# simonsysu/tfs

Measured on AMD Instinct MI355X. Metric: GiB/s CRC32 verify, device-resident 64 KiB files; 1/2/4/8 MI355X, higher is better.
Workload: dtype u8

## Files before the change

### tfs_amd/csrc/replicate_plan.h

```cpp
#pragma once
#include <algorithm>
#include <cstdint>
#include <vector>

#include "../../include/tfs_replicate.h"
#include "crc_math.h"

namespace tfscrc {

constexpr uint32_t kRepHead = 56;
constexpr uint32_t kRepOverhead = TFS_RAW_FRAME_OVERHEAD;
constexpr uint32_t kRepInfo = 36;
constexpr uint32_t kRepFlag = 0x4e534654u;
constexpr uint32_t kRepSeg = 16u << 10;
constexpr uint32_t kRepNoRec = 0xffffffffu;
constexpr int32_t kRepParameterError = -1016, kRepSizeError = -8034, kRepSizeInvalid = -16002;

struct RepUnit {
  uint64_t soff;
  uint64_t doff;
  uint32_t hlen;
  uint32_t hk;
  uint32_t plen;
  uint32_t rec;
  uint32_t frame;
  uint32_t mfh;
  uint32_t mfp;
  uint32_t mr;
};
static_assert(sizeof(RepUnit) == 48, "replicate unit layout");

struct RepFrame {
  uint64_t doff;
  uint64_t pid;
  uint32_t seed;
  uint32_t length;
  uint32_t offset;
  uint32_t flag;
  uint32_t block_id;
  uint32_t type_ver;
  uint32_t u0, nu;
};
static_assert(sizeof(RepFrame) == 48, "replicate frame layout");

struct RepRec {
  uint64_t file_id;
  int32_t offset, size;
};

struct RepPlan {
  int32_t total = 0, frame_len = 0;
  uint32_t nframes = 0;
  std::vector<RepUnit> units;
  std::vector<uint32_t> frame_first;
  std::vector<RepRec> recs;
  std::vector<uint32_t> index;
  std::vector<int32_t> early;
};

inline uint32_t rep_frame_count(int64_t total, int64_t frame_len) {
  if (total < 0 || frame_len <= 0) return 0u;
  return uint32_t(std::max<int64_t>(1, (total + frame_len - 1) / frame_len));
}

inline uint32_t rep_pow(uint64_t d) {
  struct Pow {
    uint32_t t[4][256];
    Pow() {
      for (int j = 0; j < 4; ++j) {
        t[j][0] = 1u << 31;
        const uint32_t step = shift_bytes_pow(1u << 31, uint64_t(1) << (8 * j));
        for (int v = 1; v < 256; ++v) t[j][v] = multmodp(t[j][v - 1], step);
      }
    }
  };
  static const Pow pw;
  uint32_t p = pw.t[0][d & 255u];
  for (int j = 1; j < 4; ++j)
    if ((d >> (8 * j)) & 255u) p = multmodp(p, pw.t[j][(d >> (8 * j)) & 255u]);
  return d >> 32 ? multmodp(p, shift_bytes_pow(1u << 31, d >> 32 << 32)) : p;
}

struct RepPowWalk {
  uint64_t d = 0;
  uint32_t m = 0;
  bool valid = false;
  uint32_t at(uint64_t nd) {
    struct Seg {
      uint32_t t[4][256];
      Seg() { make_shift_table(t, kRepSeg); }
    };
    static const Seg sg;
    if (valid && nd == d + kRepSeg)
      m = sg.t[0][m & 255u] ^ sg.t[1][(m >> 8) & 255u] ^ sg.t[2][(m >> 16) & 255u] ^ sg.t[3][m >> 24];
    else
      m = rep_pow(nd);
    d = nd, valid = true;
    return m;
  }
};

inline uint32_t rep_crc_bytes(uint32_t c, const uint8_t* p, uint32_t len) {
  for (uint32_t i = 0; i < len; ++i) {
    c ^= p[i];
    for (int k = 0; k < 8; ++k) c = (c & 1u) ? (c >> 1) ^ kPoly : (c >> 1);
  }
  return c;
}

inline void rep_le32(uint8_t* p, uint32_t v) {
  p[0] = uint8_t(v), p[1] = uint8_t(v >> 8), p[2] = uint8_t(v >> 16), p[3] = uint8_t(v >> 24);
}

inline void rep_info_bytes(uint32_t block_id, uint32_t offset, uint32_t length, uint8_t h[32]) {
  std::fill(h, h + 32, uint8_t(0));
  rep_le32(h, block_id);
  rep_le32(h + 12, offset);
  rep_le32(h + 16, length);
}

inline uint32_t rep_frame_seed(uint32_t block_id, uint32_t offset, uint32_t length, uint32_t flag) {
  uint8_t h[32], f[4];
  rep_info_bytes(block_id, offset, length, h);
  rep_le32(f, flag);
  return shift_bytes_pow(rep_crc_bytes(kRepFlag, h, 32), uint64_t(length) + 4u) ^ rep_crc_bytes(0u, f, 4);
}

inline int rep_cfg_status(const tfs_replicate_cfg& c) {
  if (c.total < 0 || c.frame_len <= 0 || c.frame_len % 1024 != 0) return kRepSizeInvalid;
  if (c.frame_stride != 0 && uint64_t(c.frame_stride) < uint64_t(c.frame_len) + kRepOverhead) return kRepParameterError;
  if (c.new_block != TFS_RAW_NORMAL_DATA && c.new_block != TFS_RAW_PARITY_DATA) return kRepParameterError;
  if (c.reserved != 0) return kRepParameterError;
  return 0;
}

inline uint64_t rep_stride(const tfs_replicate_cfg& c) {
  return c.frame_stride ? uint64_t(c.frame_stride) : uint64_t(c.frame_len) + kRepOverhead;
}

inline int make_replicate_plan(const tfs_replicate_cfg& c, const tfs_raw_meta* metas, uint32_t n, RepPlan* p) {
  *p = RepPlan();
  if (const int rc = rep_cfg_status(c)) return rc;
  if (n && !metas) return kRepParameterError;
  const int64_t total = c.total, fl = c.frame_len;
  p->total = c.total, p->frame_len = c.frame_len;
  p->nframes = rep_frame_count(total, fl);
  int64_t last_end = 0;
  for (uint32_t i = 0; i < n; ++i) {
    const tfs_raw_meta& m = metas[i];
    if (m.offset < 0 || int64_t(m.offset) + int64_t(m.size) > total) {
      p->early.push_back(kRepParameterError);
      continue;
    }
    if (m.size <= int32_t(kRepInfo)) {
      p->early.push_back(kRepSizeError);
      continue;
    }
    if (int64_t(m.offset) < last_end) return kRepParameterError;
    last_end = int64_t(m.offset) + int64_t(m.size);
    p->early.push_back(0);
    p->recs.push_back(RepRec{m.file_id, m.offset, m.size});
    p->index.push_back(i);
  }
  auto piece_end = [&](int64_t pos, int64_t end) {
    const int64_t fend = std::min<int64_t>((pos / fl + 1) * fl, total);
    int64_t e = std::min(end, fend);
    if (e - pos > int64_t(kRepSeg)) e = (pos / int64_t(kRepSeg) + 1) * int64_t(kRepSeg);
    return e;
  };
  auto push = [&](int64_t pos, uint32_t hlen, uint32_t hk, uint32_t plen, uint32_t rec, int64_t rec_end) {
    const int64_t fend = std::min<int64_t>((pos / fl + 1) * fl, total);
    const int64_t uend = pos + hlen + plen;
    RepUnit u{};
    u.soff = uint64_t(pos);
    u.hlen = hlen, u.hk = hk, u.plen = plen, u.rec = rec;
    u.frame = uint32_t(pos / fl);
    u.mfh = hlen ? rep_pow(uint64_t(fend - (pos + hlen)) + 4u) : 0u;
    u.mfp = uint32_t(fend - uend) + 4u;
    u.mr = rec == kRepNoRec ? 0u : uint32_t(rec_end - uend);
    p->units.push_back(u);
  };
  auto gap = [&](int64_t pos, int64_t end) {
    while (pos < end) {
      const int64_t e = piece_end(pos, end);
      push(pos, 0u, 0u, uint32_t(e - pos), kRepNoRec, 0);
      pos = e;
    }
  };
  int64_t pos = 0;
  for (uint32_t r = 0; r < uint32_t(p->recs.size()); ++r) {
    const int64_t off = p->recs[r].offset, info_end = off + kRepInfo, end = off + p->recs[r].size;
    gap(pos, off);
    pos = off;
    while (pos < end) {
      const int64_t fend = std::min<int64_t>((pos / fl + 1) * fl, total);
      uint32_t hlen = 0, hk = 0, plen = 0;
      const int64_t start = pos;
      if (pos < info_end) {
        hk = uint32_t(pos - off);
        hlen = uint32_t(std::min(info_end, fend) - pos);
        pos += hlen;
      }
      if (pos >= info_end && pos < fend) {
        plen = uint32_t(piece_end(pos, end) - pos);
        pos += plen;
      }
      push(start, hlen, hk, plen, r, end);
    }
  }
  gap(pos, total);
  RepPowWalk fw, rw;
  for (size_t k = p->units.size(); k-- > 0;) {
    RepUnit& u = p->units[k];
    u.mfp = fw.at(u.mfp);
    if (u.rec != kRepNoRec) u.mr = rw.at(u.mr);
  }
  p->frame_first.assign(size_t(p->nframes) + 1, uint32_t(p->units.size()));
  for (uint32_t k = uint32_t(p->units.size()); k-- > 0;) p->frame_first[p->units[k].frame] = k;
  for (uint32_t f = p->nframes; f-- > 0;)
    p->frame_first[f] = std::min(p->frame_first[f], p->frame_first[f + 1]);
  return 0;
}

inline bool rep_call_ok(const RepPlan& p, int64_t next, bool done, int64_t offset, int64_t len) {
  if (offset != next || len < 0) return false;
  if (p.total == 0) return !done && offset == 0 && len == 0;
  if (len == 0 || offset + len > p.total) return false;
  return offset % p.frame_len == 0 && (len % p.frame_len == 0 || offset + len == p.total);
}

inline uint32_t rep_call_frames(const RepPlan& p, int64_t len) {
  return uint32_t(std::max<int64_t>(1, (len + p.frame_len - 1) / p.frame_len));
}
inline uint64_t rep_call_need(const RepPlan& p, int64_t len, uint64_t stride) {
  const uint32_t nf = rep_call_frames(p, len);
  const uint64_t last = uint64_t(len) - uint64_t(nf - 1) * uint64_t(p.frame_len);
  return uint64_t(nf - 1) * stride + kRepOverhead + last;
}

inline uint32_t rep_slice_units(const RepPlan& p, uint32_t f0, uint32_t nf) {
  return p.frame_first[f0 + nf] - p.frame_first[f0];
}

inline void rep_make_slice(const RepPlan& p, const tfs_replicate_cfg& c, uint64_t stride, uint32_t f0, uint32_t nf,
                           RepFrame* frames, RepUnit* units) {
  const uint32_t ub = p.frame_first[f0];
  const uint64_t base = uint64_t(f0) * uint64_t(p.frame_len);
  for (uint32_t j = 0; j < nf; ++j) {
    const uint32_t f = f0 + j;
    const uint64_t off = uint64_t(f) * uint64_t(p.frame_len);
    RepFrame& fr = frames[j];
    fr.doff = uint64_t(j) * stride;
    fr.pid = c.packet_id + f;
    fr.length = uint32_t(std::min<uint64_t>(uint64_t(p.frame_len), uint64_t(p.total) - off));
    fr.offset = uint32_t(off);
    fr.flag = f == 0 ? uint32_t(int32_t(c.new_block)) : 0u;
    fr.block_id = c.block_id;
    fr.type_ver = uint32_t(TFS_WRITE_RAW_DATA_MESSAGE) | uint32_t(uint16_t(c.version)) << 16;
    fr.seed = rep_frame_seed(c.block_id, fr.offset, fr.length, fr.flag);
    fr.u0 = p.frame_first[f] - ub;
    fr.nu = p.frame_first[f + 1] - p.frame_first[f];
  }
  const uint32_t nu = rep_slice_units(p, f0, nf);
  for (uint32_t k = 0; k < nu; ++k) {
    RepUnit u = p.units[ub + k];
    const uint64_t pos = u.soff;
    const uint32_t j = u.frame - f0;
    u.soff = pos - base;
    u.doff = uint64_t(j) * stride + kRepHead + (pos - uint64_t(u.frame) * uint64_t(p.frame_len));
    u.frame = j;
    units[k] = u;
  }
}

}
```

### tfs_amd/csrc/tfs_crc_abi.cpp

```cpp
#include <emmintrin.h>
#include <hip/hip_runtime.h>

#include <algorithm>
#include <atomic>
#include <chrono>
#include <condition_variable>
#include <cstdarg>
#include <cstdio>
#include <cstdlib>
#include <cstring>
#include <map>
#include <memory>
#include <mutex>
#include <shared_mutex>
#include <string>
#include <vector>

#include "../../include/tfs_crc.h"
#include "../../include/tfs_crc_testing.h"
#include "../../include/tfs_read.h"
#include "../../include/tfs_replicate.h"
#include "../../include/tfs_write.h"
#include "crc_math.h"
#include "pin_registry.h"
// ... 204 lines not shown
  DevBuf d_src, d_dst, d_aux;
  PinBuf h_aux, h_status, h_stage;
  std::vector<uint32_t> live_idx;
  tfs_block_job* job = nullptr;
  std::vector<tfs_block_job*> gjobs;
  std::vector<uint32_t> gstart;
  std::vector<CompactJob> gjob_list;
  bool busy = false;
  void release() {
    d_src.release(); d_dst.release(); d_aux.release();
    h_aux.release(); h_status.release(); h_stage.release();
    if (done) (void)hipEventDestroy(done);
    if (stream) (void)hipStreamDestroy(stream);
    done = nullptr;
    stream = nullptr;
  }
};
struct ReadPlanSlot {
  PinBuf h;
  DevBuf d;
  hipEvent_t done = nullptr;
  void release() {
    if (done) {
      (void)hipEventSynchronize(done);
      (void)hipEventDestroy(done);
    }
    done = nullptr;
    h.release();
    d.release();
  }
};
constexpr uint32_t kReadPlanRing = 4;
struct RepRes {
  DevBuf d_cap, d_racc, d_fcrc, d_recs, d_res;
  PinBuf h_res, h_recs;
  ReadPlanSlot slots[4];
  hipEvent_t ready = nullptr;
  uint32_t slot_next = 0;
  void release() {
    for (auto& sl : slots) sl.release();
    d_cap.release(); d_racc.release(); d_fcrc.release(); d_recs.release(); d_res.release();
    h_res.release(); h_recs.release();
    if (ready) (void)hipEventDestroy(ready);
    ready = nullptr;
  }
};
constexpr size_t kRepPool = 8;
constexpr uint64_t kReadPiece = 32ull << 20;
constexpr int kCompactSlots = 8;
constexpr uint32_t kSchedSlots = 256;
constexpr uint32_t kForeignSlots = 64;
constexpr uint32_t kOwnedSlots = kSchedSlots - kForeignSlots;
constexpr int kVariantDmaCompact = 8;
#ifdef TFS_CRC_MEASURE
constexpr int kVariantStagedWide = 52;
constexpr int kVariantWideCtxStream = 53;
#else
constexpr int kVariantStagedWide = -1;
constexpr int kVariantWideCtxStream = -1;
#endif
constexpr int64_t kResRecentNs = 50'000'000;
constexpr uint64_t kZeroCopySpan = 8ull << 20;
constexpr uint32_t kZeroCopyOutFiles = 65536;

}

struct tfs_crc_ctx {
  int device = -1;
  uint64_t id = 0;
  hipStream_t stream = nullptr;
  hipStream_t lat_stream = nullptr;
  int lat_prio = 0;
  Tables* d_tables = nullptr;
  std::mutex mu;
// ... 2171 lines not shown
    HIP_TRY(ctx, hipMemcpyAsync(ctx->read_h_res.p, d_res, size_t(m) * sizeof(tfs_read_result), hipMemcpyDeviceToHost,
                                ctx->stream));
    HIP_TRY(ctx, hipStreamSynchronize(ctx->stream));
    const tfs_read_result* hr = static_cast<const tfs_read_result*>(ctx->read_h_res.p);
    for (uint32_t k = 0; k < m; ++k) {
      results[i0 + k] = hr[k];
      bad += hr[k].status != TFS_SUCCESS ? 1u : 0u;
      if (!out_zc && hr[k].frame_len)
        memcpy(o8 + jobs[i0 + k].frame_offset, static_cast<const uint8_t*>(ctx->read_h_out.p) + opos[k], hr[k].frame_len);
    }
    i0 = i1;
  }
  if (n_bad) *n_bad += bad;
  return bad ? TFS_EXIT_CHECK_CRC_ERROR : TFS_SUCCESS;
}

int tfs_read_set_piece(tfs_crc_ctx* ctx, uint64_t bytes) {
  if (!ctx) return TFS_EXIT_PARAMETER_ERROR;
  ctx->read_piece.store(bytes ? bytes : kReadPiece, std::memory_order_relaxed);
  return TFS_SUCCESS;
}


struct tfs_replicate {
  tfs_crc_ctx* ctx = nullptr;
  tfs_replicate_cfg cfg{};
  RepPlan plan;
  uint32_t n = 0;
  hipStream_t stream = nullptr;
  bool stream_set = false;
  int64_t next = 0;
  bool done = false;
  bool waited = false;
  std::unique_ptr<RepRes> r;
};

extern "C++" {
namespace {

int rep_call_checks(tfs_replicate* s, const void* src, int offset, int len, const void* out, uint64_t out_cap) {
  if (!s) return TFS_EXIT_PARAMETER_ERROR;
  if (!rep_call_ok(s->plan, s->next, s->done, offset, len))
    return set_err(s->ctx, TFS_EXIT_PARAMETER_ERROR, "replicate: call [%d, +%d) is not the next one (covered %lld of %d)",
                   offset, len, (long long)s->next, s->plan.total);
  if ((len > 0 && !src) || !out) return TFS_EXIT_DATA_INVALID;
  if (out_cap < rep_call_need(s->plan, len, rep_stride(s->cfg)))
    return set_err(s->ctx, TFS_EXIT_PARAMETER_ERROR, "replicate: out_cap does not hold the call's frames");
  return TFS_SUCCESS;
}

int rep_enqueue(tfs_replicate* s, hipStream_t st, const uint8_t* d_src, uint32_t f0, uint32_t nf, uint64_t src_len,
                uint8_t* d_out, uint64_t stride) {
  tfs_crc_ctx* ctx = s->ctx;
  RepRes& r = *s->r;
  ReadPlanSlot& rp = r.slots[r.slot_next++ % 4u];
  if (!s->waited) {
    if (st != ctx->stream) HIP_TRY(ctx, hipStreamWaitEvent(st, r.ready, 0));
    s->waited = true;
  }
  if (rp.done) HIP_TRY(ctx, hipEventSynchronize(rp.done));
  const uint32_t nu = rep_slice_units(s->plan, f0, nf);
  const size_t fbytes = size_t(nf) * sizeof(RepFrame), ubytes = size_t(nu) * sizeof(RepUnit);
  HIP_TRY(ctx, rp.h.reserve(fbytes + ubytes));
  HIP_TRY(ctx, rp.d.reserve(fbytes + ubytes + size_t(nu) * 8u));
  RepFrame* hf = static_cast<RepFrame*>(rp.h.p);
  RepUnit* hu = reinterpret_cast<RepUnit*>(static_cast<uint8_t*>(rp.h.p) + fbytes);
  rep_make_slice(s->plan, s->cfg, stride, f0, nf, hf, hu);
  uint8_t* d8 = static_cast<uint8_t*>(rp.d.p);
  const uint8_t* plan8 = static_cast<const uint8_t*>(rp.h.dev);
  if (!plan8) {
    HIP_TRY(ctx, hipMemcpyAsync(rp.d.p, rp.h.p, fbytes + ubytes, hipMemcpyHostToDevice, st));
    plan8 = d8;
  }
  SCHED_LAUNCH(ctx, st, "replicate",
               launch_replicate(d_src, src_len, reinterpret_cast<const RepUnit*>(plan8 + fbytes), nu,
                                reinterpret_cast<const RepFrame*>(plan8), nf, d_out, ctx->d_tables,
                                reinterpret_cast<uint32_t*>(d8 + fbytes + ubytes), static_cast<uint8_t*>(r.d_cap.p),
                                static_cast<uint32_t*>(r.d_racc.p), static_cast<uint32_t*>(r.d_fcrc.p) + f0, sched,
                                st, throughput_cap(ctx)));
  if (!rp.done) HIP_TRY(ctx, hipEventCreateWithFlags(&rp.done, hipEventDisableTiming));
  HIP_TRY(ctx, hipEventRecord(rp.done, st));
  return TFS_SUCCESS;
}

void rep_release(tfs_replicate* s) {
  if (!s->r) return;
  std::lock_guard<std::mutex> g(s->ctx->rep_mu);
  if (s->ctx->rep_pool.size() < kRepPool) s->ctx->rep_pool.push_back(std::move(s->r));
  else s->r->release();
  s->r.reset();
}

}
}

uint32_t tfs_replicate_frame_count(const tfs_replicate_cfg* cfg) {
  return cfg ? rep_frame_count(cfg->total, cfg->frame_len) : 0u;
}

int tfs_replicate_begin(tfs_crc_ctx* ctx, const tfs_replicate_cfg* cfg, const tfs_raw_meta* metas, uint32_t n,
                        tfs_replicate** out) {
  if (!ctx || !cfg || !out) return TFS_EXIT_PARAMETER_ERROR;
  *out = nullptr;
  std::unique_ptr<tfs_replicate> s(new tfs_replicate());
  if (const int rc = make_replicate_plan(*cfg, metas, n, &s->plan))
    return set_err(ctx, rc, "replicate begin: the configuration or the metas are refused (%d)", rc);
  s->ctx = ctx;
  s->cfg = *cfg;
  s->n = n;
  const size_t na = s->plan.recs.size();
  HIP_TRY(ctx, hipSetDevice(ctx->device));
  {
    std::lock_guard<std::mutex> g(ctx->rep_mu);
    if (!ctx->rep_pool.empty()) {
      s->r = std::move(ctx->rep_pool.back());
      ctx->rep_pool.pop_back();
    }
  }
  if (!s->r) s->r.reset(new RepRes());
  int rc = TFS_SUCCESS;
  auto setup = [&]() -> int {
    RepRes& r = *s->r;
    HIP_TRY(ctx, r.d_fcrc.reserve(size_t(s->plan.nframes) * 4u));
    HIP_TRY(ctx, r.h_res.reserve(na * 8u + size_t(s->plan.nframes) * 4u));
    if (!r.ready) HIP_TRY(ctx, hipEventCreateWithFlags(&r.ready, hipEventDisableTiming));
    if (na) {
      HIP_TRY(ctx, r.d_cap.reserve(na * kFileInfoSize));
      HIP_TRY(ctx, r.d_racc.reserve(na * 4u));
      HIP_TRY(ctx, r.d_recs.reserve(na * sizeof(RepRec)));
      HIP_TRY(ctx, r.h_recs.reserve(na * sizeof(RepRec)));
      HIP_TRY(ctx, r.d_res.reserve(na * 8u));
      memcpy(r.h_recs.p, s->plan.recs.data(), na * sizeof(RepRec));
    }
    std::lock_guard<std::mutex> g(ctx->mu);
    if (na) {
      HIP_TRY(ctx, hipMemsetAsync(r.d_racc.p, 0, na * 4u, ctx->stream));
      HIP_TRY(ctx, hipMemcpyAsync(r.d_recs.p, r.h_recs.p, na * sizeof(RepRec), hipMemcpyHostToDevice, ctx->stream));
    }
    HIP_TRY(ctx, hipEventRecord(r.ready, ctx->stream));
    return TFS_SUCCESS;
  };
  rc = setup();
  if (rc != TFS_SUCCESS) {
    rep_release(s.get());
    return rc;
  }
  *out = s.release();
  return TFS_SUCCESS;
}

int tfs_replicate_frames_device(tfs_replicate* s, const void* d_src, int offset, int len, void* d_out,
                                uint64_t out_cap, void* stream) {
  if (const int rc = rep_call_checks(s, d_src, offset, len, d_out, out_cap)) return rc;
  tfs_crc_ctx* ctx = s->ctx;
  hipStream_t st = stream ? static_cast<hipStream_t>(stream) : ctx->stream;
  if (st == hipStreamPerThread)
    return set_err(ctx, TFS_EXIT_PARAMETER_ERROR, "hipStreamPerThread is not accepted; pass NULL or a stream of your own");
  if (s->stream_set && st != s->stream)
    return set_err(ctx, TFS_EXIT_PARAMETER_ERROR, "replicate: one stream per session");
  HIP_TRY(ctx, hipSetDevice(ctx->device));
  const uint32_t f0 = uint32_t(offset / s->plan.frame_len), nf = rep_call_frames(s->plan, len);
  if (const int rc = rep_enqueue(s, st, static_cast<const uint8_t*>(d_src), f0, nf, uint64_t(len),
                                 static_cast<uint8_t*>(d_out), rep_stride(s->cfg)))
    return rc;
  s->stream = st, s->stream_set = true;
  s->next += len;
  s->done = true;
  return TFS_SUCCESS;
}

int tfs_replicate_frames(tfs_replicate* s, const void* src, int offset, int len, void* out, uint64_t out_cap) {
  if (const int rc = rep_call_checks(s, src, offset, len, out, out_cap)) return rc;
  tfs_crc_ctx* ctx = s->ctx;
  if (s->stream_set && s->stream != ctx->stream)
    return set_err(ctx, TFS_EXIT_PARAMETER_ERROR, "replicate: one stream per session");
  const uint32_t f0 = uint32_t(offset / s->plan.frame_len), nf = rep_call_frames(s->plan, len);
  {
    const Desc d0{0u, uint32_t(len), 0u};
    count_host_call(ctx, &d0, nf);
  }
  std::lock_guard<std::mutex> g(ctx->mu);
  if (const int f = injected_fault(ctx)) return f;
  HIP_TRY(ctx, hipSetDevice(ctx->device));
  void *zsrc = nullptr, *zout = nullptr;
  const bool src_zc = len == 0 || (is_pinned_host(src) && host_dev_ptr(src, &zsrc));
  const bool out_zc = is_pinned_host(out) && host_dev_ptr(out, &zout);
  (void)hipGetLastError();
  const uint64_t fl = uint64_t(s->plan.frame_len), ustride = rep_stride(s->cfg), sstride = fl + 64u;
  const uint8_t* s8 = static_cast<const uint8_t*>(src);
  uint8_t* o8 = static_cast<uint8_t*>(out);
  uint32_t per = nf;
  if (!src_zc || !out_zc) {
    const uint64_t piece = std::max<uint64_t>(ctx->read_piece.load(std::memory_order_relaxed), 1u);
    per = uint32_t(std::min<uint64_t>(nf, std::max<uint64_t>(piece / sstride, 1u)));
  }
  for (uint32_t j0 = 0; j0 < nf; j0 += per) {
    const uint32_t m = std::min(per, nf - j0);
    const uint64_t poff = uint64_t(j0) * fl;
    const uint64_t plen = std::min<uint64_t>(uint64_t(m) * fl, uint64_t(len) - poff);
    const uint8_t* d_src = static_cast<const uint8_t*>(zsrc) + poff;
// ... 5 lines not shown
      stride = sstride;
    }
    if (!src_zc) {
      HIP_TRY(ctx, ctx->read_h_src.reserve(plen + 16u));
      HIP_TRY(ctx, ctx->read_d_src.reserve(plen + 16u));
      const uintptr_t want = out_zc ? reinterpret_cast<uintptr_t>(d_out) + kRepHead : 0u;
      const uint64_t sa = (want - reinterpret_cast<uintptr_t>(ctx->read_d_src.p)) & 15u;
      memcpy(static_cast<uint8_t*>(ctx->read_h_src.p) + sa, s8 + poff, plen);
      if (plen)
        HIP_TRY(ctx, hipMemcpyAsync(static_cast<uint8_t*>(ctx->read_d_src.p) + sa,
                                    static_cast<uint8_t*>(ctx->read_h_src.p) + sa, plen, hipMemcpyHostToDevice,
                                    ctx->stream));
      d_src = static_cast<const uint8_t*>(ctx->read_d_src.p) + sa;
    }
    uint64_t oa = 0;
    if (!out_zc) {
      oa = (reinterpret_cast<uintptr_t>(d_src) - kRepHead - reinterpret_cast<uintptr_t>(ctx->read_d_out.p)) & 15u;
      d_out = static_cast<uint8_t*>(ctx->read_d_out.p) + oa;
    }
    if (const int rc = rep_enqueue(s, ctx->stream, d_src, f0 + j0, m, plen, d_out, stride)) return rc;
    const uint64_t last = plen - uint64_t(m - 1) * fl;
    if (!out_zc)
      HIP_TRY(ctx, hipMemcpyAsync(static_cast<uint8_t*>(ctx->read_h_out.p) + oa, d_out,
                                  uint64_t(m - 1) * sstride + kRepOverhead + last, hipMemcpyDeviceToHost, ctx->stream));
    HIP_TRY(ctx, hipStreamSynchronize(ctx->stream));
    if (!out_zc)
      for (uint32_t j = 0; j < m; ++j)
        memcpy(o8 + uint64_t(j0 + j) * ustride, static_cast<const uint8_t*>(ctx->read_h_out.p) + oa + uint64_t(j) * sstride,
               kRepOverhead + (j + 1 < m ? fl : last));
  }
  s->stream = ctx->stream, s->stream_set = true;
  s->next += len;
  s->done = true;
  return TFS_SUCCESS;
}

int tfs_replicate_finish(tfs_replicate* s, uint32_t* out_crc, int32_t* out_status, uint32_t* n_bad,
                         uint32_t* out_frame_crc) {
  if (!s) return TFS_EXIT_PARAMETER_ERROR;
  tfs_crc_ctx* ctx = s->ctx;
  if (!(s->plan.total == 0 ? s->done : s->next == s->plan.total))
    return set_err(ctx, TFS_EXIT_PARAMETER_ERROR, "replicate finish: %lld of %d bytes covered", (long long)s->next,
                   s->plan.total);
  HIP_TRY(ctx, hipSetDevice(ctx->device));
  hipStream_t st = s->stream_set ? s->stream : ctx->stream;
  const uint32_t na = uint32_t(s->plan.recs.size()), nfr = s->plan.nframes;
  RepRes& r = *s->r;
  if (!s->waited && st != ctx->stream) HIP_TRY(ctx, hipStreamWaitEvent(st, r.ready, 0));
  uint32_t* hr = static_cast<uint32_t*>(r.h_res.p);
  if (na) {
    uint32_t* d_crc = static_cast<uint32_t*>(r.d_res.p);
    HIP_TRY(ctx, launch_replicate_finish(static_cast<const RepRec*>(r.d_recs.p), na,
                                         static_cast<const uint8_t*>(r.d_cap.p),
                                         static_cast<const uint32_t*>(r.d_racc.p), d_crc,
                                         reinterpret_cast<int32_t*>(d_crc + na), st));
    HIP_TRY(ctx, hipMemcpyAsync(hr, d_crc, size_t(na) * 8u, hipMemcpyDeviceToHost, st));
  }
  HIP_TRY(ctx, hipMemcpyAsync(hr + 2u * size_t(na), r.d_fcrc.p, size_t(nfr) * 4u, hipMemcpyDeviceToHost, st));
  HIP_TRY(ctx, hipStreamSynchronize(st));
  uint32_t bad = 0;
  for (uint32_t i = 0; i < s->n; ++i) {
    if (out_crc) out_crc[i] = 0u;
    if (out_status) out_status[i] = s->plan.early[i];
    bad += s->plan.early[i] != 0 ? 1u : 0u;
  }
  for (uint32_t r = 0; r < na; ++r) {
    const int32_t status = int32_t(hr[na + r]);
    if (out_crc) out_crc[s->plan.index[r]] = hr[r];
    if (out_status) out_status[s->plan.index[r]] = status;
    bad += status != TFS_SUCCESS ? 1u : 0u;
  }
  if (out_frame_crc) memcpy(out_frame_crc, hr + 2u * size_t(na), size_t(nfr) * 4u);
  if (n_bad) *n_bad += bad;
  return TFS_SUCCESS;
}

int tfs_replicate_free(tfs_replicate* s) {
  if (!s) return TFS_EXIT_PARAMETER_ERROR;
  (void)hipSetDevice(s->ctx->device);
  if (s->stream_set) (void)hipStreamSynchronize(s->stream);
  if (!s->waited && s->r && s->r->ready) (void)hipEventSynchronize(s->r->ready);
  rep_release(s);
  delete s;
  return TFS_SUCCESS;
}


int tfs_crc32_shift_device(tfs_crc_ctx* ctx, const uint32_t* d_crc, const uint32_t* d_nbytes, uint32_t n,
                           uint32_t* d_out, void* stream) {
  if (!ctx || (n && (!d_crc || !d_nbytes || !d_out))) return TFS_EXIT_PARAMETER_ERROR;
  if (n == 0) return TFS_SUCCESS;
  HIP_TRY(ctx, hipSetDevice(ctx->device));
  hipStream_t st = stream ? static_cast<hipStream_t>(stream) : ctx->stream;
  HIP_TRY(ctx, launch_crc_shift(ctx->d_tables, d_crc, d_nbytes, n, d_out, st));
  return TFS_SUCCESS;
}

int tfs_crc32_synth_fill_device(tfs_crc_ctx* ctx, void* d_dst, uint64_t nbytes, uint64_t seed, uint64_t first_word,
                                void* stream) {
  if (!ctx || !d_dst || (nbytes & 7)) return TFS_EXIT_PARAMETER_ERROR;
  HIP_TRY(ctx, hipSetDevice(ctx->device));
  hipStream_t st = stream ? static_cast<hipStream_t>(stream) : ctx->stream;
  HIP_TRY(ctx, launch_synth_fill(static_cast<uint64_t*>(d_dst), nbytes / 8, seed, first_word, st));
  return TFS_SUCCESS;
}

int tfs_crc32_write_headers_device(tfs_crc_ctx* ctx, void* d_image, const uint64_t* d_rec_off, const uint32_t* d_len,
                                   const uint32_t* d_crc, uint64_t first_id, uint32_t n, void* stream) {
  if (!ctx || !d_image) return TFS_EXIT_PARAMETER_ERROR;
  HIP_TRY(ctx, hipSetDevice(ctx->device));
  hipStream_t st = stream ? static_cast<hipStream_t>(stream) : ctx->stream;
  HIP_TRY(ctx, launch_write_headers(static_cast<uint8_t*>(d_image), d_rec_off, d_len, d_crc, first_id, n, st));
  return TFS_SUCCESS;
// ... 382 lines not shown
```

### tfs_amd/csrc/tfs_crc_kernels.hip

```cpp
#include <hip/hip_runtime.h>
#include <stdint.h>

#include <type_traits>

#include "read_reply_plan.h"
#include "replicate_plan.h"
#include "tfs_crc_device.h"

namespace tfscrc {

typedef const __attribute__((address_space(1))) uint32_t* gu32p;
typedef unsigned int u32x4 __attribute__((ext_vector_type(4)));
typedef const __attribute__((address_space(1))) u32x4* gu128p;
typedef const __attribute__((address_space(1))) uint8_t* gu8p;
__device__ __forceinline__ uint32_t ld32(uintptr_t a) { return *reinterpret_cast<gu32p>(a); }
__device__ __forceinline__ uint4 ld128(uintptr_t a) {
  const u32x4 v = *reinterpret_cast<gu128p>(a);
  return make_uint4(v.x, v.y, v.z, v.w);
}
template <bool NT>
__device__ __forceinline__ uint4 ld128s(uintptr_t a) {
  if (NT) {
    const u32x4 v = __builtin_nontemporal_load(reinterpret_cast<gu128p>(a));
    return make_uint4(v.x, v.y, v.z, v.w);
  }
  return ld128(a);
}
__device__ __forceinline__ uint32_t ld8(uintptr_t a) { return *reinterpret_cast<gu8p>(a); }

__device__ __forceinline__ uint32_t xor3(uint32_t a, uint32_t b, uint32_t c) {
  return __builtin_amdgcn_bitop3_b32(a, b, c, 0x96);
}

__device__ __forceinline__ uint32_t lds_ld(const uint32_t* T, uint32_t byte_addr) {
  return *reinterpret_cast<const uint32_t*>(reinterpret_cast<const char*>(T) + byte_addr);
// ... 1920 lines not shown
      }
      if (uint32_t(lane) < cur.hlen) {
        out[cur.doff + uint32_t(lane)] = uint8_t(st.hb);
        cap[uint64_t(cur.rec) * kFileInfoSize + cur.hk + uint32_t(lane)] = uint8_t(st.hb);
      }
      if (st.g.nstripes) {
        if (lane == 0) {
          const uint32_t ntw = uint32_t((st.g.end & ~uintptr_t(3)) - st.g.B16) / 4u;
          for (uint32_t i = 0; i < 3u; ++i)
            if (i < ntw) st32u(st.g.B16 + 4u * i + st.delta, st.h.tw[i]);
          const uintptr_t B = st.g.end & ~uintptr_t(3);
          for (uint32_t i = 0; i < 3u; ++i)
            if (B + i < st.g.end) *reinterpret_cast<uint8_t*>(B + i + st.delta) = uint8_t(st.h.tb[i]);
        }
      } else {
        copy_unaligned(src + cur.soff + cur.hlen, out + cur.doff + cur.hlen, cur.plen, lane);
      }
      c = finish_file<kRun, kLY>(lds_tables, lb, st.g, st.h, c, lane);
      const uint32_t ch = cur.hlen ? rep_info_crc(lds_tables, lb, st.hb, cur.hlen) : 0u;
      if (lane == 0) {
        ucrc[2u * f] = ch;
        ucrc[2u * f + 1u] = c;
      }
      if (!more) break;
      f = fn;
      fn = fnn;
      cur = ncur;
      st = ns;
    }
  } while (false);
  if (lane == 0) launch_exit(sched, gridDim.x * wpb, nullptr, 0u);
}

__device__ __forceinline__ uint32_t gf_mul(uint32_t a, uint32_t b) {
  uint32_t p = 0u;
#pragma unroll 4
  for (uint32_t i = 0; i < 32u; ++i) {
    p ^= (a & (0x80000000u >> i)) ? b : 0u;
    b = (b >> 1) ^ ((b & 1u) ? kPoly : 0u);
  }
  return p;
}

__global__ void __launch_bounds__(kWave) replicate_fold_kernel(const RepFrame* __restrict__ frames,
                                                               const RepUnit* __restrict__ units,
                                                               const uint32_t* __restrict__ ucrc,
                                                               uint8_t* __restrict__ out, uint32_t* racc,
                                                               uint32_t* __restrict__ fcrc) {
  const RepFrame fr = frames[blockIdx.x];
  const uint32_t lane = threadIdx.x;
  uint32_t x = 0u;
  for (uint32_t k = lane; k < fr.nu; k += kWave) {
    const RepUnit u = units[fr.u0 + k];
    const uint32_t ch = ucrc[2u * (fr.u0 + k)], cp = ucrc[2u * (fr.u0 + k) + 1u];
    x ^= gf_mul(u.mfh, ch) ^ gf_mul(u.mfp, cp);
    if (u.rec != kRepNoRec && u.plen) atomicXor(&racc[u.rec], gf_mul(u.mr, cp));
  }
#pragma unroll
  for (int m = kWave / 2; m >= 1; m >>= 1) x ^= __shfl_xor(x, m, kWave);
  const uint32_t crc = int16_t(uint16_t(fr.type_ver >> 16)) < 1 ? 0u : fr.seed ^ x;
  if (lane == 0) fcrc[blockIdx.x] = crc;
  uint8_t* frame = out + fr.doff;
  if (lane < kRepHead) {
    const uint32_t k = lane >> 2;
    const uint32_t w = k == 0u    ? kPacketFlagV1
                       : k == 1u  ? kRepInfo + fr.length
                       : k == 2u  ? fr.type_ver
                       : k == 3u  ? uint32_t(fr.pid)
                       : k == 4u  ? uint32_t(fr.pid >> 32)
                       : k == 5u  ? crc
                       : k == 6u  ? fr.block_id
                       : k == 9u  ? fr.offset
                       : k == 10u ? fr.length
                                  : 0u;
    frame[lane] = uint8_t(w >> (8u * (lane & 3u)));
  } else if (lane < kRepOverhead) {
    frame[kRepHead + fr.length + (lane - kRepHead)] = uint8_t(fr.flag >> (8u * (lane & 3u)));
  }
}

__global__ void __launch_bounds__(256) replicate_finish_kernel(const RepRec* __restrict__ recs, uint32_t n,
                                                               const uint8_t* __restrict__ cap,
                                                               const uint32_t* __restrict__ racc,
                                                               uint32_t* __restrict__ out_crc,
                                                               int32_t* __restrict__ out_status) {
  const uint32_t i = blockIdx.x * blockDim.x + threadIdx.x;
  if (i >= n) return;
  const uint8_t* fi = cap + uint64_t(i) * kFileInfoSize;
  const RepRec r = recs[i];
  const uint64_t id = uint64_t(ld_le32(fi)) | uint64_t(ld_le32(fi + 4)) << 32;
  const uint32_t c = racc[i];
  int32_t status = kSuccess;
  if (id != r.file_id) status = kExitFileInfoError;
  else if (int32_t(ld_le32(fi + 12)) != r.size) status = kExitSyncFileError;
  else if (c != ld_le32(fi + 32)) status = kExitCheckCrcError;
  out_crc[i] = c;
  out_status[i] = status;
}

__global__ void __launch_bounds__(256) compact_seg_plan_kernel(const CompactJob* __restrict__ jobs, uint32_t n,
                                                               uint64_t src_len, CSegArgs cs) {
  __shared__ uint32_t wsum[4];
  __shared__ unsigned long long blk_base;
  const uint32_t i = blockIdx.x * 256u + threadIdx.x;
  const int lane = threadIdx.x & (kWave - 1);
  const uint32_t w = threadIdx.x / kWave;
  const uint32_t seg = 1024u << cs.lg;
  CompactJob j{};
  uint32_t K = 0;
  if (i < n) {
// ... 680 lines not shown
  if (variant == 50 && jobs) TFS_BV(true, 1, 0);
  else if (variant == 50) TFS_BV(false, 1, 0);
  else
#endif
  if (jobs) TFS_BV(true, kCF, kTS);
  else TFS_BV(false, kCF, kTS);
#undef TFS_BV
  (void)variant;
  return hipGetLastError();
}

hipError_t launch_read_reply(const uint8_t* src, uint64_t src_len, const ReadUnit* units, uint32_t n, uint8_t* out,
                             const Tables* tg, ReadResult* results, uint32_t* n_bad, uint32_t* sched,
                             hipStream_t stream, unsigned cap) {
  if (n == 0) return hipSuccess;
  if (!sched) return hipErrorInvalidValue;
  hipLaunchKernelGGL(read_reply_kernel, dim3(grid_for(n, cap)), dim3(kBlock), 0, stream, src, src_len, units, n, out,
                     tg, results, n_bad, sched);
  return hipGetLastError();
}

hipError_t launch_replicate(const uint8_t* src, uint64_t src_len, const RepUnit* units, uint32_t nu,
                            const RepFrame* frames, uint32_t nf, uint8_t* out, const Tables* tg, uint32_t* ucrc,
                            uint8_t* cap_bytes, uint32_t* racc, uint32_t* fcrc, uint32_t* sched, hipStream_t stream,
                            unsigned cap) {
  if (nf == 0) return hipSuccess;
  if (nu) {
    if (!sched) return hipErrorInvalidValue;
    hipLaunchKernelGGL(replicate_kernel, dim3(grid_for(nu, cap)), dim3(kBlock), 0, stream, src, src_len, units, nu, out,
                       tg, ucrc, cap_bytes, sched);
    const hipError_t e = hipGetLastError();
    if (e != hipSuccess) return e;
  }
  hipLaunchKernelGGL(replicate_fold_kernel, dim3(nf), dim3(kWave), 0, stream, frames, units, ucrc, out, racc, fcrc);
  return hipGetLastError();
}

hipError_t launch_replicate_finish(const RepRec* recs, uint32_t n, const uint8_t* cap_bytes, const uint32_t* racc,
                                   uint32_t* out_crc, int32_t* out_status, hipStream_t stream) {
  if (n == 0) return hipSuccess;
  hipLaunchKernelGGL(replicate_finish_kernel, dim3((n + 255u) / 256u), dim3(256), 0, stream, recs, n, cap_bytes, racc,
                     out_crc, out_status);
  return hipGetLastError();
}

hipError_t launch_synth_fill(uint64_t* dst, uint64_t nwords, uint64_t seed, uint64_t first_word, hipStream_t stream) {
  if (nwords == 0) return hipSuccess;
  uint64_t g = (nwords + 255) / 256;
  if (g > 65536) g = 65536;
  hipLaunchKernelGGL(synth_fill_kernel, dim3(unsigned(g)), dim3(256), 0, stream, dst, nwords, seed, first_word);
  return hipGetLastError();
}

#ifdef TFS_CRC_MEASURE
template <int PF, int SK, int HOLE = 0>
__global__ void __launch_bounds__(kBlock) membench_copy_chunk_kernel(const uint8_t* __restrict__ src,
                                                                     uint8_t* __restrict__ dst, uint64_t nbytes,
                                                                     uint64_t ch) {
  const int lane = threadIdx.x & (kWave - 1);
  const uint64_t wave = uint64_t(blockIdx.x) * (kBlock / kWave) + __builtin_amdgcn_readfirstlane(threadIdx.x / kWave);
  const uint64_t nw = uint64_t(gridDim.x) * (kBlock / kWave);
  const uint64_t nch = nbytes / ch;
  const uintptr_t s = reinterpret_cast<uintptr_t>(src), d = reinterpret_cast<uintptr_t>(dst);
  for (uint64_t c = wave; c < nch; c += nw) {
    const uint64_t b = c * ch + 16u * uint64_t(lane);
    for (uint64_t o = 0; o < ch; o += 1024u * PF) {
      uint4 v[PF];
// ... 92 lines not shown
```

Measured before the change: 6218.

## Move CRC shift powers from host plan to device fold using shift tables

The replicate plan no longer computes GF(2) multipliers on the host for each unit. It stores raw byte distances instead, and the fold kernel applies them on the GPU with the level shift tables cached in LDS. The fold kernel now packs several frames per 256-thread block and accumulates them through shared atomics. Other changes reuse pooled plan vectors, fuse the two device-to-host result copies into one, and skip a redundant stream sync on free. The cost moves from host planning to per-item shift loops on the device, which can be long for large distances.

```diff
diff --git a/tfs_amd/csrc/replicate_plan.h b/tfs_amd/csrc/replicate_plan.h
--- a/tfs_amd/csrc/replicate_plan.h
+++ b/tfs_amd/csrc/replicate_plan.h
@@ -13,6 +13,7 @@
 constexpr uint32_t kRepInfo = 36;
 constexpr uint32_t kRepFlag = 0x4e534654u;
 constexpr uint32_t kRepSeg = 16u << 10;
+static_assert((kRepSeg & (kRepSeg - 1u)) == 0u, "the walk cuts at multiples of kRepSeg with a mask");
 constexpr uint32_t kRepNoRec = 0xffffffffu;
 constexpr int32_t kRepParameterError = -1016, kRepSizeError = -8034, kRepSizeInvalid = -16002;
 
@@ -24,9 +25,9 @@
   uint32_t plen;
   uint32_t rec;
   uint32_t frame;
-  uint32_t mfh;
-  uint32_t mfp;
-  uint32_t mr;
+  uint32_t dfh;
+  uint32_t dfp;
+  uint32_t dr;
 };
 static_assert(sizeof(RepUnit) == 48, "replicate unit layout");
 
@@ -56,6 +57,10 @@
   std::vector<RepRec> recs;
   std::vector<uint32_t> index;
   std::vector<int32_t> early;
+  void reset() {
+    total = frame_len = 0, nframes = 0;
+    units.clear(), frame_first.clear(), recs.clear(), index.clear(), early.clear();
+  }
 };
 
 inline uint32_t rep_frame_count(int64_t total, int64_t frame_len) {
@@ -63,48 +68,13 @@
   return uint32_t(std::max<int64_t>(1, (total + frame_len - 1) / frame_len));
 }
 
-inline uint32_t rep_pow(uint64_t d) {
-  struct Pow {
-    uint32_t t[4][256];
-    Pow() {
-      for (int j = 0; j < 4; ++j) {
-        t[j][0] = 1u << 31;
-        const uint32_t step = shift_bytes_pow(1u << 31, uint64_t(1) << (8 * j));
-        for (int v = 1; v < 256; ++v) t[j][v] = multmodp(t[j][v - 1], step);
-      }
-    }
-  };
-  static const Pow pw;
-  uint32_t p = pw.t[0][d & 255u];
-  for (int j = 1; j < 4; ++j)
-    if ((d >> (8 * j)) & 255u) p = multmodp(p, pw.t[j][(d >> (8 * j)) & 255u]);
-  return d >> 32 ? multmodp(p, shift_bytes_pow(1u << 31, d >> 32 << 32)) : p;
-}
-
-struct RepPowWalk {
-  uint64_t d = 0;
-  uint32_t m = 0;
-  bool valid = false;
-  uint32_t at(uint64_t nd) {
-    struct Seg {
-      uint32_t t[4][256];
-      Seg() { make_shift_table(t, kRepSeg); }
-    };
-    static const Seg sg;
-    if (valid && nd == d + kRepSeg)
-      m = sg.t[0][m & 255u] ^ sg.t[1][(m >> 8) & 255u] ^ sg.t[2][(m >> 16) & 255u] ^ sg.t[3][m >> 24];
-    else
-      m = rep_pow(nd);
-    d = nd, valid = true;
-    return m;
-  }
-};
-
 inline uint32_t rep_crc_bytes(uint32_t c, const uint8_t* p, uint32_t len) {
-  for (uint32_t i = 0; i < len; ++i) {
-    c ^= p[i];
-    for (int k = 0; k < 8; ++k) c = (c & 1u) ? (c >> 1) ^ kPoly : (c >> 1);
-  }
+  struct Tab {
+    uint32_t t[256];
+    Tab() { make_byte_table(t); }
+  };
+  static const Tab tb;
+  for (uint32_t i = 0; i < len; ++i) c = (c >> 8) ^ tb.t[(c ^ p[i]) & 0xffu];
   return c;
 }
 
@@ -119,11 +89,15 @@
   rep_le32(h + 16, length);
 }
 
-inline uint32_t rep_frame_seed(uint32_t block_id, uint32_t offset, uint32_t length, uint32_t flag) {
+inline uint32_t rep_seed_pow(uint32_t length) { return shift_bytes_pow(1u << 31, uint64_t(length) + 4u); }
+inline uint32_t rep_frame_seed(uint32_t block_id, uint32_t offset, uint32_t length, uint32_t flag, uint32_t pow) {
   uint8_t h[32], f[4];
   rep_info_bytes(block_id, offset, length, h);
   rep_le32(f, flag);
-  return shift_bytes_pow(rep_crc_bytes(kRepFlag, h, 32), uint64_t(length) + 4u) ^ rep_crc_bytes(0u, f, 4);
+  return multmodp(pow, rep_crc_bytes(kRepFlag, h, 32)) ^ rep_crc_bytes(0u, f, 4);
+}
+inline uint32_t rep_frame_seed(uint32_t block_id, uint32_t offset, uint32_t length, uint32_t flag) {
+  return rep_frame_seed(block_id, offset, length, flag, rep_seed_pow(length));
 }
 
 inline int rep_cfg_status(const tfs_replicate_cfg& c) {
@@ -139,12 +113,13 @@
 }
 
 inline int make_replicate_plan(const tfs_replicate_cfg& c, const tfs_raw_meta* metas, uint32_t n, RepPlan* p) {
-  *p = RepPlan();
+  p->reset();
   if (const int rc = rep_cfg_status(c)) return rc;
   if (n && !metas) return kRepParameterError;
   const int64_t total = c.total, fl = c.frame_len;
   p->total = c.total, p->frame_len = c.frame_len;
   p->nframes = rep_frame_count(total, fl);
+  p->early.reserve(n), p->recs.reserve(n), p->index.reserve(n);
   int64_t last_end = 0;
   for (uint32_t i = 0; i < n; ++i) {
     const tfs_raw_meta& m = metas[i];
@@ -162,23 +137,29 @@
     p->recs.push_back(RepRec{m.file_id, m.offset, m.size});
     p->index.push_back(i);
   }
+  p->units.reserve(size_t(p->nframes) + size_t(total / int64_t(kRepSeg)) + 2u * p->recs.size() + 2u);
+  p->frame_first.assign(size_t(p->nframes) + 1, 0u);
+  uint32_t f = 0;
+  int64_t fend = std::min(fl, total);
   auto piece_end = [&](int64_t pos, int64_t end) {
-    const int64_t fend = std::min<int64_t>((pos / fl + 1) * fl, total);
     int64_t e = std::min(end, fend);
-    if (e - pos > int64_t(kRepSeg)) e = (pos / int64_t(kRepSeg) + 1) * int64_t(kRepSeg);
+    if (e - pos > int64_t(kRepSeg)) e = (pos & ~int64_t(kRepSeg - 1u)) + int64_t(kRepSeg);
     return e;
   };
   auto push = [&](int64_t pos, uint32_t hlen, uint32_t hk, uint32_t plen, uint32_t rec, int64_t rec_end) {
-    const int64_t fend = std::min<int64_t>((pos / fl + 1) * fl, total);
     const int64_t uend = pos + hlen + plen;
-    RepUnit u{};
-    u.soff = uint64_t(pos);
+    RepUnit u;
+    u.soff = uint64_t(pos), u.doff = 0;
     u.hlen = hlen, u.hk = hk, u.plen = plen, u.rec = rec;
-    u.frame = uint32_t(pos / fl);
-    u.mfh = hlen ? rep_pow(uint64_t(fend - (pos + hlen)) + 4u) : 0u;
-    u.mfp = uint32_t(fend - uend) + 4u;
-    u.mr = rec == kRepNoRec ? 0u : uint32_t(rec_end - uend);
+    u.frame = f;
+    u.dfh = hlen ? uint32_t(fend - (pos + hlen)) + 4u : 0u;
+    u.dfp = uint32_t(fend - uend) + 4u;
+    u.dr = rec == kRepNoRec ? 0u : uint32_t(rec_end - uend);
     p->units.push_back(u);
+    if (uend == fend && uend < total) {
+      fend = std::min(fend + fl, total);
+      p->frame_first[++f] = uint32_t(p->units.size());
+    }
   };
   auto gap = [&](int64_t pos, int64_t end) {
     while (pos < end) {
@@ -193,7 +174,6 @@
     gap(pos, off);
     pos = off;
     while (pos < end) {
-      const int64_t fend = std::min<int64_t>((pos / fl + 1) * fl, total);
       uint32_t hlen = 0, hk = 0, plen = 0;
       const int64_t start = pos;
       if (pos < info_end) {
@@ -209,16 +189,7 @@
     }
   }
   gap(pos, total);
-  RepPowWalk fw, rw;
-  for (size_t k = p->units.size(); k-- > 0;) {
-    RepUnit& u = p->units[k];
-    u.mfp = fw.at(u.mfp);
-    if (u.rec != kRepNoRec) u.mr = rw.at(u.mr);
-  }
-  p->frame_first.assign(size_t(p->nframes) + 1, uint32_t(p->units.size()));
-  for (uint32_t k = uint32_t(p->units.size()); k-- > 0;) p->frame_first[p->units[k].frame] = k;
-  for (uint32_t f = p->nframes; f-- > 0;)
-    p->frame_first[f] = std::min(p->frame_first[f], p->frame_first[f + 1]);
+  p->frame_first[p->nframes] = uint32_t(p->units.size());
   return 0;
 }
 
@@ -246,6 +217,7 @@
                            RepFrame* frames, RepUnit* units) {
   const uint32_t ub = p.frame_first[f0];
   const uint64_t base = uint64_t(f0) * uint64_t(p.frame_len);
+  const uint32_t full_pow = rep_seed_pow(uint32_t(p.frame_len));
   for (uint32_t j = 0; j < nf; ++j) {
     const uint32_t f = f0 + j;
     const uint64_t off = uint64_t(f) * uint64_t(p.frame_len);
@@ -257,7 +229,8 @@
     fr.flag = f == 0 ? uint32_t(int32_t(c.new_block)) : 0u;
     fr.block_id = c.block_id;
     fr.type_ver = uint32_t(TFS_WRITE_RAW_DATA_MESSAGE) | uint32_t(uint16_t(c.version)) << 16;
-    fr.seed = rep_frame_seed(c.block_id, fr.offset, fr.length, fr.flag);
+    fr.seed = rep_frame_seed(c.block_id, fr.offset, fr.length, fr.flag,
+                             fr.length == uint32_t(p.frame_len) ? full_pow : rep_seed_pow(fr.length));
     fr.u0 = p.frame_first[f] - ub;
     fr.nu = p.frame_first[f + 1] - p.frame_first[f];
   }
diff --git a/tfs_amd/csrc/tfs_crc_abi.cpp b/tfs_amd/csrc/tfs_crc_abi.cpp
--- a/tfs_amd/csrc/tfs_crc_abi.cpp
+++ b/tfs_amd/csrc/tfs_crc_abi.cpp
@@ -260,14 +260,15 @@
 };
 constexpr uint32_t kReadPlanRing = 4;
 struct RepRes {
-  DevBuf d_cap, d_racc, d_fcrc, d_recs, d_res;
+  DevBuf d_cap, d_racc, d_recs, d_res;
   PinBuf h_res, h_recs;
+  RepPlan plan;
   ReadPlanSlot slots[4];
   hipEvent_t ready = nullptr;
   uint32_t slot_next = 0;
   void release() {
     for (auto& sl : slots) sl.release();
-    d_cap.release(); d_racc.release(); d_fcrc.release(); d_recs.release(); d_res.release();
+    d_cap.release(); d_racc.release(); d_recs.release(); d_res.release();
     h_res.release(); h_recs.release();
     if (ready) (void)hipEventDestroy(ready);
     ready = nullptr;
@@ -2505,7 +2506,9 @@
   int64_t next = 0;
   bool done = false;
   bool waited = false;
+  bool drained = false;
   std::unique_ptr<RepRes> r;
+  uint32_t* d_fcrc() const { return static_cast<uint32_t*>(r->d_res.p) + 2u * plan.recs.size(); }
 };
 
 extern "C++" {
@@ -2549,7 +2552,7 @@
                launch_replicate(d_src, src_len, reinterpret_cast<const RepUnit*>(plan8 + fbytes), nu,
                                 reinterpret_cast<const RepFrame*>(plan8), nf, d_out, ctx->d_tables,
                                 reinterpret_cast<uint32_t*>(d8 + fbytes + ubytes), static_cast<uint8_t*>(r.d_cap.p),
-                                static_cast<uint32_t*>(r.d_racc.p), static_cast<uint32_t*>(r.d_fcrc.p) + f0, sched,
+                                static_cast<uint32_t*>(r.d_racc.p), s->d_fcrc() + f0, sched,
                                 st, throughput_cap(ctx)));
   if (!rp.done) HIP_TRY(ctx, hipEventCreateWithFlags(&rp.done, hipEventDisableTiming));
   HIP_TRY(ctx, hipEventRecord(rp.done, st));
@@ -2558,6 +2561,8 @@
 
 void rep_release(tfs_replicate* s) {
   if (!s->r) return;
+  std::swap(s->plan, s->r->plan);
+  s->r->plan.reset();
   std::lock_guard<std::mutex> g(s->ctx->rep_mu);
   if (s->ctx->rep_pool.size() < kRepPool) s->ctx->rep_pool.push_back(std::move(s->r));
   else s->r->release();
@@ -2576,13 +2581,7 @@
   if (!ctx || !cfg || !out) return TFS_EXIT_PARAMETER_ERROR;
   *out = nullptr;
   std::unique_ptr<tfs_replicate> s(new tfs_replicate());
-  if (const int rc = make_replicate_plan(*cfg, metas, n, &s->plan))
-    return set_err(ctx, rc, "replicate begin: the configuration or the metas are refused (%d)", rc);
   s->ctx = ctx;
-  s->cfg = *cfg;
-  s->n = n;
-  const size_t na = s->plan.recs.size();
-  HIP_TRY(ctx, hipSetDevice(ctx->device));
   {
     std::lock_guard<std::mutex> g(ctx->rep_mu);
     if (!ctx->rep_pool.empty()) {
@@ -2591,10 +2590,19 @@
     }
   }
   if (!s->r) s->r.reset(new RepRes());
+  std::swap(s->plan, s->r->plan);
+  if (const int rc = make_replicate_plan(*cfg, metas, n, &s->plan)) {
+    rep_release(s.get());
+    return set_err(ctx, rc, "replicate begin: the configuration or the metas are refused (%d)", rc);
+  }
+  s->cfg = *cfg;
+  s->n = n;
+  const size_t na = s->plan.recs.size();
   int rc = TFS_SUCCESS;
   auto setup = [&]() -> int {
     RepRes& r = *s->r;
-    HIP_TRY(ctx, r.d_fcrc.reserve(size_t(s->plan.nframes) * 4u));
+    HIP_TRY(ctx, hipSetDevice(ctx->device));
+    HIP_TRY(ctx, r.d_res.reserve(na * 8u + size_t(s->plan.nframes) * 4u));
     HIP_TRY(ctx, r.h_res.reserve(na * 8u + size_t(s->plan.nframes) * 4u));
     if (!r.ready) HIP_TRY(ctx, hipEventCreateWithFlags(&r.ready, hipEventDisableTiming));
     if (na) {
@@ -2602,7 +2610,6 @@
       HIP_TRY(ctx, r.d_racc.reserve(na * 4u));
       HIP_TRY(ctx, r.d_recs.reserve(na * sizeof(RepRec)));
       HIP_TRY(ctx, r.h_recs.reserve(na * sizeof(RepRec)));
-      HIP_TRY(ctx, r.d_res.reserve(na * 8u));
       memcpy(r.h_recs.p, s->plan.recs.data(), na * sizeof(RepRec));
     }
     std::lock_guard<std::mutex> g(ctx->mu);
@@ -2639,6 +2646,7 @@
   s->stream = st, s->stream_set = true;
   s->next += len;
   s->done = true;
+  s->drained = false;
   return TFS_SUCCESS;
 }
 
@@ -2710,6 +2718,7 @@
   s->stream = ctx->stream, s->stream_set = true;
   s->next += len;
   s->done = true;
+  s->drained = false;
   return TFS_SUCCESS;
 }
 
@@ -2725,28 +2734,25 @@
   const uint32_t na = uint32_t(s->plan.recs.size()), nfr = s->plan.nframes;
   RepRes& r = *s->r;
   if (!s->waited && st != ctx->stream) HIP_TRY(ctx, hipStreamWaitEvent(st, r.ready, 0));
-  uint32_t* hr = static_cast<uint32_t*>(r.h_res.p);
-  if (na) {
-    uint32_t* d_crc = static_cast<uint32_t*>(r.d_res.p);
+  const uint32_t* hr = static_cast<const uint32_t*>(r.h_res.p);
+  uint32_t* d_crc = static_cast<uint32_t*>(r.d_res.p);
+  s->drained = false;
+  if (na)
     HIP_TRY(ctx, launch_replicate_finish(static_cast<const RepRec*>(r.d_recs.p), na,
                                          static_cast<const uint8_t*>(r.d_cap.p),
                                          static_cast<const uint32_t*>(r.d_racc.p), d_crc,
                                          reinterpret_cast<int32_t*>(d_crc + na), st));
-    HIP_TRY(ctx, hipMemcpyAsync(hr, d_crc, size_t(na) * 8u, hipMemcpyDeviceToHost, st));
-  }
-  HIP_TRY(ctx, hipMemcpyAsync(hr + 2u * size_t(na), r.d_fcrc.p, size_t(nfr) * 4u, hipMemcpyDeviceToHost, st));
+  HIP_TRY(ctx, hipMemcpyAsync(r.h_res.p, d_crc, size_t(na) * 8u + size_t(nfr) * 4u, hipMemcpyDeviceToHost, st));
   HIP_TRY(ctx, hipStreamSynchronize(st));
-  uint32_t bad = 0;
+  s->drained = true;
+  uint32_t bad = 0, k = 0;
   for (uint32_t i = 0; i < s->n; ++i) {
-    if (out_crc) out_crc[i] = 0u;
-    if (out_status) out_status[i] = s->plan.early[i];
-    bad += s->plan.early[i] != 0 ? 1u : 0u;
-  }
-  for (uint32_t r = 0; r < na; ++r) {
-    const int32_t status = int32_t(hr[na + r]);
-    if (out_crc) out_crc[s->plan.index[r]] = hr[r];
-    if (out_status) out_status[s->plan.index[r]] = status;
+    const int32_t early = s->plan.early[i];
+    const int32_t status = early ? early : int32_t(hr[na + k]);
+    if (out_crc) out_crc[i] = early ? 0u : hr[k];
+    if (out_status) out_status[i] = status;
     bad += status != TFS_SUCCESS ? 1u : 0u;
+    k += early ? 0u : 1u;
   }
   if (out_frame_crc) memcpy(out_frame_crc, hr + 2u * size_t(na), size_t(nfr) * 4u);
   if (n_bad) *n_bad += bad;
@@ -2756,7 +2762,7 @@
 int tfs_replicate_free(tfs_replicate* s) {
   if (!s) return TFS_EXIT_PARAMETER_ERROR;
   (void)hipSetDevice(s->ctx->device);
-  if (s->stream_set) (void)hipStreamSynchronize(s->stream);
+  if (s->stream_set && !s->drained) (void)hipStreamSynchronize(s->stream);
   if (!s->waited && s->r && s->r->ready) (void)hipEventSynchronize(s->r->ready);
   rep_release(s);
   delete s;
diff --git a/tfs_amd/csrc/tfs_crc_kernels.hip b/tfs_amd/csrc/tfs_crc_kernels.hip
--- a/tfs_amd/csrc/tfs_crc_kernels.hip
+++ b/tfs_amd/csrc/tfs_crc_kernels.hip
@@ -1,6 +1,7 @@
 #include <hip/hip_runtime.h>
 #include <stdint.h>
 
+#include <cstddef>
 #include <type_traits>
 
 #include "read_reply_plan.h"
@@ -1987,50 +1988,89 @@
   if (lane == 0) launch_exit(sched, gridDim.x * wpb, nullptr, 0u);
 }
 
-__device__ __forceinline__ uint32_t gf_mul(uint32_t a, uint32_t b) {
-  uint32_t p = 0u;
-#pragma unroll 4
-  for (uint32_t i = 0; i < 32u; ++i) {
-    p ^= (a & (0x80000000u >> i)) ? b : 0u;
-    b = (b >> 1) ^ ((b & 1u) ? kPoly : 0u);
-  }
-  return p;
-}
-
-__global__ void __launch_bounds__(kWave) replicate_fold_kernel(const RepFrame* __restrict__ frames,
-                                                               const RepUnit* __restrict__ units,
-                                                               const uint32_t* __restrict__ ucrc,
-                                                               uint8_t* __restrict__ out, uint32_t* racc,
-                                                               uint32_t* __restrict__ fcrc) {
-  const RepFrame fr = frames[blockIdx.x];
-  const uint32_t lane = threadIdx.x;
-  uint32_t x = 0u;
-  for (uint32_t k = lane; k < fr.nu; k += kWave) {
-    const RepUnit u = units[fr.u0 + k];
-    const uint32_t ch = ucrc[2u * (fr.u0 + k)], cp = ucrc[2u * (fr.u0 + k) + 1u];
-    x ^= gf_mul(u.mfh, ch) ^ gf_mul(u.mfp, cp);
-    if (u.rec != kRepNoRec && u.plen) atomicXor(&racc[u.rec], gf_mul(u.mr, cp));
-  }
-#pragma unroll
-  for (int m = kWave / 2; m >= 1; m >>= 1) x ^= __shfl_xor(x, m, kWave);
-  const uint32_t crc = int16_t(uint16_t(fr.type_ver >> 16)) < 1 ? 0u : fr.seed ^ x;
-  if (lane == 0) fcrc[blockIdx.x] = crc;
-  uint8_t* frame = out + fr.doff;
-  if (lane < kRepHead) {
-    const uint32_t k = lane >> 2;
-    const uint32_t w = k == 0u    ? kPacketFlagV1
-                       : k == 1u  ? kRepInfo + fr.length
-                       : k == 2u  ? fr.type_ver
-                       : k == 3u  ? uint32_t(fr.pid)
-                       : k == 4u  ? uint32_t(fr.pid >> 32)
-                       : k == 5u  ? crc
-                       : k == 6u  ? fr.block_id
-                       : k == 9u  ? fr.offset
-                       : k == 10u ? fr.length
-                                  : 0u;
-    frame[lane] = uint8_t(w >> (8u * (lane & 3u)));
-  } else if (lane < kRepOverhead) {
-    frame[kRepHead + fr.length + (lane - kRepHead)] = uint8_t(fr.flag >> (8u * (lane & 3u)));
+constexpr uint32_t kRepFoldBlock = 256;
+constexpr uint32_t kRepFoldFrames = 1024;
+static_assert(offsetof(Tables, any_shift) % 16 == 0 && (uint32_t(kAnyLevels) * kAnyStride) % 16u == 0,
+              "the fold loads the level tables 16 bytes a lane");
+
+__device__ __forceinline__ uint32_t rep_shift(const uint32_t* L, uint32_t c, uint32_t d) {
+#pragma unroll 1
+  for (uint32_t k = 0; k < uint32_t(kAnyLevels) && (d >> k) != 0u; ++k)
+    if ((d >> k) & 1u) c = shift5(L, k * kAnyStride, c);
+#pragma unroll 1
+  for (uint32_t t = 2u * (d >> kAnyLevels); t; --t) c = shift5(L, uint32_t(kAnyLevels - 1) * kAnyStride, c);
+  return c;
+}
+
+struct RepShift {
+  uint32_t c, d;
+  uint32_t to;
+  bool rec, live;
+};
+__device__ __forceinline__ RepShift rep_item(const RepUnit* __restrict__ units, const uint32_t* __restrict__ ucrc,
+                                             uint32_t ub, uint32_t n, uint32_t i) {
+  const uint32_t w = i / n, q = ub + (i - w * n);
+  const RepUnit u = units[q];
+  RepShift s;
+  s.c = ucrc[2u * q + (w == 2u ? 0u : 1u)];
+  s.d = w == 0u ? u.dfp : w == 1u ? u.dr : u.dfh;
+  s.rec = w == 1u;
+  s.to = s.rec ? u.rec : u.frame;
+  s.live = w == 0u ? true : w == 1u ? (u.rec != kRepNoRec && u.plen != 0u) : u.dfh != 0u;
+  return s;
+}
+
+__global__ void __launch_bounds__(kRepFoldBlock) replicate_fold_kernel(const RepFrame* __restrict__ frames,
+                                                                       const RepUnit* __restrict__ units,
+                                                                       const uint32_t* __restrict__ ucrc,
+                                                                       uint8_t* __restrict__ out, uint32_t* racc,
+                                                                       uint32_t* __restrict__ fcrc,
+                                                                       const Tables* __restrict__ tg, uint32_t nf,
+                                                                       uint32_t per) {
+  __shared__ uint4 L4[uint32_t(kAnyLevels) * kAnyStride / 16u];
+  __shared__ uint32_t facc[kRepFoldFrames];
+  const uint32_t* L = reinterpret_cast<const uint32_t*>(L4);
+  const uint32_t j0 = blockIdx.x * per, j1 = min(nf, j0 + per);
+  const uint4* g4 = reinterpret_cast<const uint4*>(&tg->any_shift[0][0][0]);
+  const uint32_t ub = frames[j0].u0, n = frames[j1 - 1u].u0 + frames[j1 - 1u].nu - ub;
+  uint32_t i = threadIdx.x;
+  RepShift s{};
+  if (i < 3u * n) s = rep_item(units, ucrc, ub, n, i);
+  for (uint32_t k = threadIdx.x; k < uint32_t(kAnyLevels) * kAnyStride / 16u; k += kRepFoldBlock) L4[k] = g4[k];
+  for (uint32_t k = threadIdx.x; k < j1 - j0; k += kRepFoldBlock) facc[k] = 0u;
+  __syncthreads();
+  while (i < 3u * n) {
+    if (s.live) {
+      const uint32_t x = rep_shift(L, s.c, s.d);
+      if (s.rec) atomicXor(&racc[s.to], x);
+      else atomicXor(&facc[s.to - j0], x);
+    }
+    i += kRepFoldBlock;
+    if (i < 3u * n) s = rep_item(units, ucrc, ub, n, i);
+  }
+  __syncthreads();
+  const uint32_t lane = threadIdx.x & (kWave - 1);
+  for (uint32_t j = j0 + threadIdx.x / kWave; j < j1; j += kRepFoldBlock / kWave) {
+    const RepFrame fr = frames[j];
+    const uint32_t crc = int16_t(uint16_t(fr.type_ver >> 16)) < 1 ? 0u : fr.seed ^ facc[j - j0];
+    if (lane == 0) fcrc[j] = crc;
+    uint8_t* frame = out + fr.doff;
+    if (lane < kRepHead) {
+      const uint32_t k = lane >> 2;
+      const uint32_t w = k == 0u    ? kPacketFlagV1
+                         : k == 1u  ? kRepInfo + fr.length
+                         : k == 2u  ? fr.type_ver
+                         : k == 3u  ? uint32_t(fr.pid)
+                         : k == 4u  ? uint32_t(fr.pid >> 32)
+                         : k == 5u  ? crc
+                         : k == 6u  ? fr.block_id
+                         : k == 9u  ? fr.offset
+                         : k == 10u ? fr.length
+                                    : 0u;
+      frame[lane] = uint8_t(w >> (8u * (lane & 3u)));
+    } else if (lane < kRepOverhead) {
+      frame[kRepHead + fr.length + (lane - kRepHead)] = uint8_t(fr.flag >> (8u * (lane & 3u)));
+    }
   }
 }
 
@@ -2777,7 +2817,10 @@
     const hipError_t e = hipGetLastError();
     if (e != hipSuccess) return e;
   }
-  hipLaunchKernelGGL(replicate_fold_kernel, dim3(nf), dim3(kWave), 0, stream, frames, units, ucrc, out, racc, fcrc);
+  const uint64_t fill = nu ? uint64_t(kRepFoldBlock) * nf / (3u * uint64_t(nu)) : nf;
+  const uint32_t per = uint32_t(std::min<uint64_t>(std::max<uint64_t>(fill, 1u), kRepFoldFrames));
+  hipLaunchKernelGGL(replicate_fold_kernel, dim3((nf + per - 1u) / per), dim3(kRepFoldBlock), 0, stream, frames, units,
+                     ucrc, out, racc, fcrc, tg, nf, per);
   return hipGetLastError();
 }
 
```

Measured after the change: 6243 (median of 2 runs). No clear change (+0.4%).
